# tmbdev/clstm

Hardware: AMD Instinct MI355X
Metric: text-line images/sec (fwd+bwd+CTC), 100-unit BiLSTM H=48 T~200 (higher is better)
Workload: dtype f32 (operand-exact split): forward, recurrences, CTC, decode in f32 arithmetic; the backward weight-gradient / softmax-backward products take their f32 operands split EXACTLY into three bf16 terms each (x1 + x2 + x3 = x) and sum the six bf16-MFMA products of weight >= 2^-16 in f32 -- what is dropped

## Files before the change

### clstm_amd/csrc/dbgopt.h

```cpp
#pragma once
#include <cstdlib>
#include <cstring>
#include <map>
#include <stdexcept>
#include <string>

namespace clstm {
struct DbgOptDef { const char* name; int dflt; };
inline constexpr DbgOptDef DBG_OPTS[] = {
    {"gemm_stag", 2},
    {"bwd_c32", 1},
    {"rec_x3", 1},
    {"pack_tiles", 1},
    {"fuse_wx", 1},
    {"gemm_b16mc", 1},
    {"dw_x3", 1},
    {"gemm_x3", 1},
    {"split_terms", 3},
    {"xd_prologue", 1},
    {"fwd_mfma", 1},
    {"bwd_mfma", 1},
    {"bwd_mfma_fused", 1},
    {"ctc_float", 0},
    {"peer_two_phase", 1},
};
inline const DbgOptDef* dbg_opt_def(const char* name) {
  for (const DbgOptDef& o : DBG_OPTS)
    if (strcmp(o.name, name) == 0) return &o;
  return nullptr;
}
inline std::map<std::string, int>& dbg_opts() {
  static std::map<std::string, int> m = [] {
    std::map<std::string, int> r;
    const char* e = getenv("CLSTM_DEBUG");
    if (e) {
      std::string s(e);
      size_t i = 0;
      while (i < s.size()) {
        size_t j = s.find(',', i);
        if (j == std::string::npos) j = s.size();
        const std::string kv = s.substr(i, j - i);
        const size_t eq = kv.find('=');
        if (!kv.empty()) {
          const std::string name = kv.substr(0, eq);
          if (eq == std::string::npos || !dbg_opt_def(name.c_str()))
            throw std::runtime_error("CLSTM_DEBUG: unknown option '" + name + "' (clstm_amd/csrc/dbgopt.h lists them as name=value)");
          r[name] = atoi(kv.c_str() + eq + 1);
        }
        i = j + 1;
      }
    }
    return r;
// ... 12 lines not shown
```

### clstm_amd/csrc/gemm_dw.h

```cpp
#pragma once
#include <type_traits>
#include "gemm_bf16.h"

namespace clstm {

struct DwSlab {
  int tile_begin, ntiles;
  int need_it;
  int dir;
  int out_z;
  int pad[3];
};

struct XdArgs {
  GemmOperand A;
  GemmOperand B;
  float* out; int ld;
  int K;
};

struct GemmDwArgs {
  const float* S; long long sdir; int lds; long long s_elems;
  const float* D; int M; int no4; long long d_elems;
  const int* ktab;
  int ntiles_max;
  const DwSlab* slabs;
  int nslabs;
  const int* prog;
  const int* line_off;
  int bs, prog_base, ndir;
  float* partial;
  int R, Cn;
  unsigned gx, gy;
  int* timeouts;
  int* minprog;
  int tcap;
  int* done;
  int done_target;
  long long* trace;
  int trace_base;
  const float* xS; int xlds; long long xs_elems;
  const float* xD; int xM; long long xd_elems;
  const int* xtab; const DwSlab* xslabs; int xnslabs;
  float* xpartial; int xR, xCn; unsigned xgx, xgy;
  int x3;
  int terms;
  XdArgs xd;
};

constexpr int DW_PF = 3;
constexpr int DW_STAB_MAX = 256;
// ... 337 lines not shown
```

### clstm_amd/csrc/lstm_bwd_dw.h

```cpp
#pragma once
#include "gemm_dw.h"
#include "lstm_seq.h"
#include "lstm_xd_prologue.h"

namespace clstm {

constexpr int DW_FUSED_STAB_ENTRIES = 1024;
static_assert(DW_FUSED_STAB_ENTRIES >= DW_STAB_MAX, "the items' k-tile table fits");
static_assert(xd_smem_floats(2) <= dw_img_floats(2) && xd_smem_floats(3) <= dw_img_floats(3), "the recurrence role's x.d prologue stages in the items' carve");

template <int NK4, int KU, int NT>
__global__ __launch_bounds__(64 * NK4) CLSTM_TWO_WAVES_PER_SIMD void lstm_bwd_dw_kernel(LstmSeqArgs a, GemmDwArgs g, int nrec) {
  __shared__ __attribute__((aligned(16))) float gsm[dw_img_floats(NT) + 2 * DW_FUSED_STAB_ENTRIES];
  if ((int)blockIdx.x < nrec) {
#ifndef CLSTM_HIP_EMU
    __builtin_amdgcn_s_setprio(3);
#endif
    const long long t0 = g.trace ? wall_clock() : 0;
    const int bl = (int)blockIdx.x % a.bs;
    const int b = a.order ? a.order[bl] : bl, dir = (int)blockIdx.x / a.bs;
    if constexpr (NT >= 2) {
      if (g.xd.A.p) xd_prologue<NT, xd_maxu(NK4)>(gsm, g.xd, a.line_off, b, dir, a.no);
    }
    lstm_bwd_body<NK4, KU>(a, b, dir);
    if (g.done && threadIdx.x == 0) atomic_add_i32(g.done, 1);
    if (g.trace && threadIdx.x == 0) { g.trace[blockIdx.x * 4] = t0; g.trace[blockIdx.x * 4 + 2] = wall_clock(); }
  } else {
    if (threadIdx.x >= 256) return;
    gemm_dw_body<NT>(g, gsm, blockIdx.x - (unsigned)nrec);
  }
}

}
```

### clstm_amd/csrc/lstm_seq.h

```cpp
#pragma once
#include <type_traits>
#include "devintrin.h"

namespace clstm {

struct LstmSeqArgs {
  const float* Rpk;
  float* G;
  float* C;
  float* H;
  int ldh, hofs;
  const float* dH;
  float* D;
  const int* line_off;
  const int* order;
  int no;
  int ndir;
  float* S;
  int lds, sofs;
  long long sdir;
  long long* prof;
  long long prog_off;
  int prog_base;
  int bs;
// ... 213 lines not shown
    step(t, gxA, rdyA, rdA, wrA, kaA0, kaA1, kaA2, kaB0, kaB1, kaB2);
    step(t + 1, gxB, rdyB, rdB, wrB, kaB0, kaB1, kaB2, kaA0, kaA1, kaA2);
  }
  if (t < T) {
    step(t, gxA, rdyA, rdA, wrA, kaA0, kaA1, kaA2, kaB0, kaB1, kaB2);
    if constexpr (!EARLY || STAG) flush(t, kaA0, kaA1, kaA2, report_tag);
  } else {
    if constexpr (!EARLY || STAG) flush(t - 1, kaB0, kaB1, kaB2, report_tag);
  }
  if constexpr (STAG && EARLY) __syncthreads();
  };
  if constexpr (FUSED) {
    if (wave_uniform(wave) == 3) run(std::true_type{}, std::true_type{}, std::false_type{});
    else if (early) run(std::true_type{}, std::false_type{}, std::false_type{});
    else if (wave_uniform(wave) == (nthreads >> 6) - 1) run(std::false_type{}, std::false_type{}, std::true_type{});
    else run(std::false_type{}, std::false_type{}, std::false_type{});
    drain_vmem();
    __syncthreads();
    if (tid == 0) store_i32_wt(reinterpret_cast<int*>(a.H + a.prog_off) + ((size_t)dir * a.bs + b) * PROG_STRIDE, a.prog_base + T);
  } else {
    if (early) run(std::true_type{}, std::false_type{}, std::false_type{}); else run(std::false_type{}, std::false_type{}, std::false_type{});
  }
#ifdef CLSTM_LSTM_PROF
  if (a.prof && b == 0 && dir == 0 && lane == 0)
    for (int k = 0; k < 12; k++) a.prof[wave * 12 + k] = pacc[k];
#endif
}
#undef LSTM_PIN3
template <int NK4, int KU, bool SAVE = true>
__global__ __launch_bounds__(64 * NK4) CLSTM_TWO_WAVES_PER_SIMD void lstm_fwd_kernel(LstmSeqArgs a) {
  lstm_fwd_body<NK4, KU, false, SAVE>(a, a.order ? a.order[blockIdx.x] : (int)blockIdx.x, blockIdx.y, nullptr);
}

template <int NK4, int KU>
DEVFN void lstm_bwd_body(const LstmSeqArgs& a, const int b, const int dir) {
  constexpr int SLP = 4 * NK4;
  constexpr int QS = SLP + ((NK4 & 1) ? 0 : 4);
  constexpr int DB = 16 * QS;
  float* lds = dyn_smem<float>();
  const int tid = threadIdx.x, lane = tid & 63, wave = tid >> 6;
  const int nthreads = blockDim.x;
  const int no = a.no, nd = a.ndir;
  const int SL = (4 * no + 15) / 16;
  const int js = lane & 15;
  const int g = lane & 3, cell = wave * 16 + (lane >> 2);
  const bool valid = cell < no;

  f32x2 wb01[SLP], wb23[SLP];
  {
    const float* rp = a.Rpk + (size_t)dir * 4 * SLP * nthreads + tid;
#pragma unroll
    for (int pp = 0; pp < SLP; pp++) {
      wb01[pp] = (f32x2){rp[(size_t)(0 * SLP + pp) * nthreads], rp[(size_t)(1 * SLP + pp) * nthreads]};
      wb23[pp] = (f32x2){rp[(size_t)(2 * SLP + pp) * nthreads], rp[(size_t)(3 * SLP + pp) * nthreads]};
    }
  }
  for (int i = tid; i < 2 * DB + 4; i += nthreads) lds[i] = 0.0f;

  const int off = a.line_off[b];
  const int T = a.line_off[b + 1] - off;
  if (T <= 0) {
    if (a.prog_off >= 0 && tid == 0) {
      store_i32_wt(reinterpret_cast<int*>(a.D + a.prog_off) + ((size_t)dir * a.bs + b) * PROG_STRIDE, a.prog_base);
    }
    return;
  }
  const int pidx = g * no + cell;
  const int dslot = (pidx / SL) * QS + (pidx % SL);
  const unsigned gstride4 = (unsigned)nd * 4 * no * 4, cstride4 = (unsigned)nd * no * 4;
  const BufF32 gbuf = make_buf(a.G + (size_t)off * (gstride4 / 4), (size_t)T * gstride4);
  const bool report = a.prog_off >= 0;
  const bool tagl = report && tid == nthreads - 1;
  const long long prog_rel = a.prog_off + ((long long)dir * a.bs + b) * PROG_STRIDE - (long long)off * (gstride4 / 4);
  const BufF32 dbuf = make_buf(a.D + (size_t)off * (gstride4 / 4), report ? (size_t)(prog_rel + 1) * 4 : (size_t)T * gstride4);
  const BufF32 cbuf = make_buf(a.C + (size_t)off * (cstride4 / 4), (size_t)T * cstride4);
  const BufF32 hbuf = make_buf(a.dH + (size_t)off * (cstride4 / 4), (size_t)T * cstride4);
  const unsigned gl = valid ? ((unsigned)dir * 4 * no + cell * 4 + g) * 4u : BUF_OOB_BASE;
  const unsigned ptag = (unsigned)(prog_rel * 4);
  const unsigned cl = valid ? ((unsigned)dir * no + cell) * 4u : BUF_OOB_BASE;
  auto fr = [&](int s) -> unsigned {
    const int sc = s > 0 ? s : 0;
    return (unsigned)(dir == 0 ? sc : T - 1 - sc);
  };
  const float* rdA = lds + js * QS;
  const float* rdB = lds + DB + js * QS;
  float* wrA = valid ? lds + DB + dslot : lds + 2 * DB;
  float* wrB = valid ? lds + dslot : lds + 2 * DB;
  const bool gb1 = (g & 2) != 0, gb0 = (g & 1) != 0;

  struct Ops { float act, dh, cc; };
  Ops X0, X1, X2;
  X0.act = buf_load(gbuf, gl + fr(T - 1) * gstride4); X1.act = buf_load(gbuf, gl + fr(T - 2) * gstride4);
  X0.dh = buf_load(hbuf, cl + fr(T - 1) * cstride4);  X1.dh = buf_load(hbuf, cl + fr(T - 2) * cstride4);
  X0.cc = buf_load(cbuf, cl + fr(T - 1) * cstride4);  X1.cc = buf_load(cbuf, T >= 2 ? cl + fr(T - 2) * cstride4 : BUF_OOB);
  X2.act = X2.dh = X2.cc = 0.0f;
  float dc_carry = 0.0f;
  float ka0 = 0.f, ka1 = 0.f, ka2 = 0.f;
  __syncthreads();
  auto step = [&](const int s, Ops& cur, const Ops& nxt, Ops& ld, const float* dq, float* dw, float& ka, float& kprev) {
    KEEP_ALIVE(ka);
    ld.act = buf_load(gbuf, gl + fr(s - 2) * gstride4);
    ld.dh = buf_load(hbuf, cl + fr(s - 2) * cstride4);
    ld.cc = buf_load(cbuf, s >= 2 ? cl + fr(s - 2) * cstride4 : BUF_OOB);
    const float actr = cur.act;
    const float deriv = fmaf(-actr, actr, g == 3 ? 1.0f : actr);
    const float th = tanh_fast(cur.cc);
    const float gth = mul_quad_bcast<2>(actr, fmaf(-th, th, 1.0f));
    float c_m1 = nxt.cc;
    OPAQUE(c_m1);
    const float mir = quad_mirror(actr);
    const float mid = gb0 ? c_m1 : th;
    float fb = deriv * (gb0 == gb1 ? mir : mid);
    OPAQUE(fb);
    f32x2 a01 = splat2(0.0f), a23 = splat2(0.0f);
    float4 dv[NK4];
#pragma unroll
    for (int j = 0; j < NK4; j++) dv[j] = *reinterpret_cast<const float4*>(dq + 4 * j);
    SCHED_FENCE();
    buf_store_wt(dbuf, s + 1 < T ? (tagl ? ptag : gl + fr(s + 1) * gstride4) : BUF_OOB, kprev);
    SCHED_FENCE();
#pragma unroll
    for (int j = 0; j < NK4; j++) {
      if (4 * j < KU) { a01 = fma2(wb01[4 * j], splat2(dv[j].x), a01); a23 = fma2(wb23[4 * j], splat2(dv[j].x), a23); }
      if (4 * j + 1 < KU) { a01 = fma2(wb01[4 * j + 1], splat2(dv[j].y), a01); a23 = fma2(wb23[4 * j + 1], splat2(dv[j].y), a23); }
      if (4 * j + 2 < KU) { a01 = fma2(wb01[4 * j + 2], splat2(dv[j].z), a01); a23 = fma2(wb23[4 * j + 2], splat2(dv[j].z), a23); }
      if (4 * j + 3 < KU) { a01 = fma2(wb01[4 * j + 3], splat2(dv[j].w), a01); a23 = fma2(wb23[4 * j + 3], splat2(dv[j].w), a23); }
    }
    const float k0 = a01[0] + row_ror<8>(a23[0]);
    const float k1 = a01[1] + row_ror<8>(a23[1]);
    float k = k0 + row_half_mirror(k1);
    k += quad_xor1(k);
    k += quad_xor2(k);
    const float dh = cur.dh + k;
    const float dc = dc_carry + gth * dh;
    dc_carry = mul_quad_bcast_old<1>(actr, dc);
    const float delta = (g == 2 ? dh : dc) * fb;
    const float sdat = tagl ? __builtin_bit_cast(float, a.prog_base + (T - 1 - s) - 3) : delta;
    *dw = delta;
    ka = sdat;
    __syncthreads();
  };
  int s = T - 1;
  for (; s >= 5; s -= 6) {
    step(s, X0, X1, X2, rdA, wrA, ka0, ka2);
    step(s - 1, X1, X2, X0, rdB, wrB, ka1, ka0);
    step(s - 2, X2, X0, X1, rdA, wrA, ka2, ka1);
    step(s - 3, X0, X1, X2, rdB, wrB, ka0, ka2);
    step(s - 4, X1, X2, X0, rdA, wrA, ka1, ka0);
    step(s - 5, X2, X0, X1, rdB, wrB, ka2, ka1);
  }
  if (s >= 0) step(s, X0, X1, X2, rdA, wrA, ka0, ka2);
  if (s >= 1) step(s - 1, X1, X2, X0, rdB, wrB, ka1, ka0);
  if (s >= 2) step(s - 2, X2, X0, X1, rdA, wrA, ka2, ka1);
  if (s >= 3) step(s - 3, X0, X1, X2, rdB, wrB, ka0, ka2);
  if (s >= 4) step(s - 4, X1, X2, X0, rdA, wrA, ka1, ka0);
  {
    const int r = (T - 1) % 3;
    const float last = r == 0 ? ka0 : r == 1 ? ka1 : ka2;
    buf_store_wt(dbuf, tagl ? ptag : gl + fr(0) * gstride4, last);
  }
  if (report) {
    drain_vmem();
    __syncthreads();
    if (tagl) buf_store_wt(dbuf, ptag, __builtin_bit_cast(float, a.prog_base + T));
  }
}
template <int NK4, int KU>
__global__ __launch_bounds__(64 * NK4) CLSTM_TWO_WAVES_PER_SIMD void lstm_bwd_kernel(LstmSeqArgs a) {
  lstm_bwd_body<NK4, KU>(a, a.order ? a.order[blockIdx.x] : (int)blockIdx.x, blockIdx.y);
}

}
```

### clstm_amd/csrc/lstm_xd_prologue.h

```cpp
#pragma once
#include "gemm_dw.h"
#include "lstm_seq.h"

namespace clstm {

constexpr int XD_KB = 3;
constexpr int XD_MAX_K = 32 * XD_KB;
constexpr int XD_ROWS = 32;
constexpr int XD_UNITS = XD_ROWS * XD_KB * 4;
constexpr int XD_RING = 3;
constexpr int xd_maxu(int nk4) { return nk4 <= 1 ? 6 : nk4 == 2 ? 3 : nk4 <= 7 ? 2 : 1; }
constexpr int xd_smem_floats(int nt) { return 2 * nt * XD_KB * XD_ROWS * 32 / 2; }

template <int NT, int MAXU>
DEVFN void xd_prologue(float* smem, const XdArgs& x, const int* line_off, const int b, const int dir, const int no) {
  static_assert(NT == 2 || NT == 3, "two or three bf16 terms per operand");
  unsigned short* img = reinterpret_cast<unsigned short*>(smem);
  const int tid = threadIdx.x, lane = tid & 63, wave = wave_uniform(tid >> 6);
  const int nthreads = blockDim.x;
  const int off = line_off[b];
  const int T = line_off[b + 1] - off;
  if (T <= 0) return;
  const int K = x.K;
  const BufF32 abuf = make_buf(x.A.p + (size_t)off * x.A.ld, (size_t)(x.A.elems - (long long)off * x.A.ld) * 4);
  const BufF32 bbuf = make_buf(x.B.p, (size_t)x.B.elems * 4);
  const BufF32 obuf = make_buf(x.out + (size_t)off * x.ld, (size_t)T * x.ld * 4);
  const int fk = lane >> 4, fi = lane & 15;
  constexpr int IMG = XD_ROWS * 32;
  constexpr int BUFH = NT * XD_KB * IMG;

  auto load_round = [&](const int r, f32x4 (&ra)[MAXU][2]) {
#pragma unroll
    for (int i = 0; i < MAXU; i++) {
      if (i * nthreads + (tid & ~63) >= XD_UNITS) break;
      const int u = i * nthreads + tid;
      const int row = r * XD_ROWS + u / (XD_KB * 4), ku = u % (XD_KB * 4);
      const unsigned o = u < XD_UNITS && row < T ? ((unsigned)row * (unsigned)x.A.ld + (unsigned)((ku >> 2) * 32 + (ku & 3) * 8)) * 4u : BUF_OOB_BASE;
      ra[i][0] = buf_load4(abuf, o);
      ra[i][1] = buf_load4(abuf, o + 16u);
    }
  };
  auto stage_round = [&](unsigned short* dst, const f32x4 (&ra)[MAXU][2]) {
#pragma unroll
    for (int i = 0; i < MAXU; i++) {
      if (i * nthreads + (tid & ~63) >= XD_UNITS) break;
      const int u = i * nthreads + tid;
      if (u < XD_UNITS) {
        const int row = u / (XD_KB * 4), ku = u % (XD_KB * 4), kb = ku >> 2, kk = (ku & 3) * 8;
        float v[8];
#pragma unroll
        for (int e = 0; e < 8; e++) v[e] = kb * 32 + kk + e < K ? ra[i][e >> 2][e & 3] : 0.0f;
        const int o = kb * IMG + row * 32 + (((kk >> 3) ^ gb2_sw(row)) << 3);
#pragma unroll
        for (int t = 0; t < NT; t++) {
          const u16x8 h = bf16_pack8(v);
          *reinterpret_cast<u16x8*>(dst + t * XD_KB * IMG + o) = h;
          if (t + 1 < NT) {
#pragma unroll
            for (int e = 0; e < 8; e++) v[e] -= __builtin_bit_cast(float, (unsigned)h[e] << 16);
          }
        }
      }
    }
  };

  f32x4 ring[XD_RING][MAXU][2];
#pragma unroll
  for (int p = 0; p < XD_RING; p++) {
    load_round(p, ring[p]);
    SCHED_FENCE();
  }

  const int n = wave * 16 + fi;
  const bool has_tile = wave * 16 < no;
  u16x8 bt[XD_KB][NT];
  if (has_tile) {
    const unsigned brow = n < no ? (unsigned)(dir * no + n) * (unsigned)x.B.ld * 4u : BUF_OOB_BASE;
    f32x4 rb[XD_KB][2];
#pragma unroll
    for (int kb = 0; kb < XD_KB; kb++) {
      rb[kb][0] = buf_load4(bbuf, brow + (unsigned)(kb * 32 + fk * 8) * 4u);
      rb[kb][1] = buf_load4(bbuf, brow + (unsigned)(kb * 32 + fk * 8 + 4) * 4u);
    }
#pragma unroll
    for (int kb = 0; kb < XD_KB; kb++) {
      float v[8];
#pragma unroll
      for (int i = 0; i < 8; i++) v[i] = kb * 32 + fk * 8 + i < K ? rb[kb][i >> 2][i & 3] : 0.0f;
#pragma unroll
      for (int t = 0; t < NT; t++) {
        const u16x8 h = bf16_pack8(v);
        bt[kb][t] = h;
        if (t + 1 < NT) {
#pragma unroll
          for (int i = 0; i < 8; i++) v[i] -= __builtin_bit_cast(float, (unsigned)h[i] << 16);
        }
      }
    }
  }

  const int nrounds = (T + XD_ROWS - 1) / XD_ROWS;
  const int fofs = fi * 32 + ((fk ^ gb2_sw(fi)) << 3);
  const unsigned ocol = n < no ? (unsigned)(dir * no + n) * 4u : BUF_OOB_BASE;
  auto round = [&](const int r, f32x4 (&ra)[MAXU][2]) {
    unsigned short* cur = img + (r & 1) * BUFH;
    stage_round(cur, ra);
    wait_lgkmcnt0();
    wg_barrier();
    COMPILER_MEMORY_BARRIER();
    load_round(r + XD_RING, ra);
    SCHED_FENCE();
    if (has_tile) {
      f32x4 acc[2];
#pragma unroll
      for (int m = 0; m < 2; m++)
#pragma unroll
        for (int q = 0; q < 4; q++) acc[m][q] = 0.0f;
#pragma unroll
      for (int kb = 0; kb < XD_KB; kb++) {
        u16x8 at[NT][2];
#pragma unroll
        for (int t = 0; t < NT; t++)
#pragma unroll
          for (int m = 0; m < 2; m++) at[t][m] = *reinterpret_cast<const u16x8*>(cur + (t * XD_KB + kb) * IMG + m * 16 * 32 + fofs);
#pragma unroll
        for (int w = NT - 1; w >= 0; w--)
#pragma unroll
          for (int ta = w; ta >= 0; ta--)
#pragma unroll
            for (int m = 0; m < 2; m++) acc[m] = mfma16x16x32_bf16(at[ta][m], bt[kb][w - ta], acc[m]);
      }
#pragma unroll
      for (int m = 0; m < 2; m++)
#pragma unroll
        for (int q = 0; q < 4; q++) {
          const int row = r * XD_ROWS + m * 16 + fk * 4 + q;
          buf_store(obuf, row < T ? (unsigned)row * (unsigned)x.ld * 4u + ocol : BUF_OOB_BASE, acc[m][q]);
        }
    }
  };
  for (int r = 0; r < nrounds; r += XD_RING) {
#pragma unroll
    for (int p = 0; p < XD_RING; p++)
      if (r + p < nrounds) round(r + p, ring[p]);
  }
  drain_vmem();
  __syncthreads();
}

template <int NK4, int KU, int NT>
__global__ __launch_bounds__(64 * NK4) CLSTM_TWO_WAVES_PER_SIMD void lstm_bwd_xd_kernel(LstmSeqArgs a, XdArgs x) {
  __shared__ __attribute__((aligned(16))) float xsm[xd_smem_floats(NT)];
  const int b = a.order ? a.order[blockIdx.x] : (int)blockIdx.x;
  xd_prologue<NT, xd_maxu(NK4)>(xsm, x, a.line_off, b, (int)blockIdx.y, a.no);
  lstm_bwd_body<NK4, KU>(a, b, (int)blockIdx.y);
}

}
```

### clstm_amd/csrc/net.inc

```
struct Layer {
  int ni, no, nk4, nthreads;
  bool wide = false;
  int kpf = 0, kpb = 0;
  long long nwf = 0, nwb = 0;
  PackDesc pd;
  float *Wt = nullptr, *bias = nullptr, *Rf = nullptr, *Rb = nullptr, *Rwf = nullptr, *Rwb = nullptr;
  float* Wk = nullptr;
  int wk_kp = 0, wk_njp = 0;
  DevBuf<float> dCc;
  DevBuf<unsigned short> Wmf;
  DevBuf<float> mf_scale;
  DevBuf<unsigned> mf_xmax;
  long long mf_epoch = -1;
  DevBuf<unsigned short> Wmfb;
  long long mfb_epoch = -1;
  DevBuf<int> pack_tab;
  DevBuf<int> pack_inv;
  int pack_inv_state = 0;
  unsigned short *Rbf = nullptr, *Rbb = nullptr;
  DevBuf<unsigned short> R2b, D2;
  bool r2b_ready = false;
  DevBuf<unsigned short> Hb, Db;
  DevBuf<float> Rf32;
  long long* moff = nullptr;
// ... 47 lines not shown
  bool bf16_rec = false;
  bool want_dx0 = false;
  int bs = 0, tmax = 0;
  bool src0_ready = false;
  long long N = 0;
  std::vector<int> line_off_h;
  DevBuf<int> line_off;
  std::vector<int> order_h;
  PinnedRing ring;
  const int* lo_stage = nullptr;
  bool lo_pending = false;
  void flush_line_off() {
    if (!lo_pending) return;
    hipStream_t s = stream();
    HIPCHECK(hipMemcpyAsync(line_off.p, lo_stage, (2 * bs + 1) * sizeof(int), hipMemcpyHostToDevice, s));
    ring.commit(s);
    lo_pending = false;
  }
  DevBuf<float> X, Z, Dz, dX0, partial, partial_sm, aligned, tmp;
  DevBuf<unsigned short> xbf;
  ReduceDesc sm_red{};
  DevBuf<long long> lstm_prof;
  StepGraphCache step_graphs;
  DevBuf<int> coop_sync;
  DevBuf<int> states, state_off, dec_idx, dec_cls, dec_loc, dec_cnt;
  DevBuf<float> dec_val, lat;
  DevBuf<long long> lat_off;
  Timing timing;
  static const int PROG_LINES = 2048;
  static const int PROG_WORDS = 2 * PROG_LINES * PROG_STRIDE;
  int overlap = getenv("CLSTM_OVERLAP") ? atoi(getenv("CLSTM_OVERLAP")) : 1;
  unsigned dw_done_total = 0;
  DevBuf<long long> dw_trace;
  DevBuf<int> dw_ktab, dw_slabs, dw_queue;
  std::vector<int> dw_key;
  DevBuf<int> dwx_tab;
  long long dwx_N = -1;
  int dwx_nslabs = 0, dwx_entries = 0;
  bool dwx_active = false;
  int dw_nslabs = 0, dw_slabs_per_dir = 0, dw_ntiles_max = 0;
  int prog_base = 1024;
  long long dw_launches = 0;
  Comm* comm = nullptr;
  struct HostFeed {
    hipStream_t cs = nullptr;
    hipEvent_t copied[2] = {};
    DevBuf<float> xin[2];
    void* pin[2] = {nullptr, nullptr};
    size_t pin_cap[2] = {0, 0};
    int* step_done = nullptr;
    long long steps = 0;
    bool ready = false;
  } hf;
  float* W1k = nullptr;
  int w1k_kps = 0;
  DevBuf<int> fw_items, fw_flags;
  std::vector<int> fw_key;
  int fw_npitems = 0, fw_ncitems = 0, fw_chunks = 0;
  int fw_epoch = 0, fw_prog_base = 1024;
  long long fw_launches = 0;

  hipStream_t stream() const { return g_stream; }
  bool geom_predict = false, nosave = false, in_predict = false;
  size_t fixed_bytes = 0;
  void dev_malloc(void** q, size_t bytes) { HIPCHECK(hipMalloc(q, bytes)); fixed_bytes += bytes; }

// ... 732 lines not shown
  bool dw_x3 = dbg_opt("dw_x3") != 0;
  int split_terms = dbg_opt("split_terms");
  bool gemm_x3_on = dbg_opt("gemm_x3") != 0;
  bool strict_f32 = false;
  bool rec_x3() const {
    if (bf16_gemm || bf16_rec || !gemm_x3_on) return false;
    return dbg_opt("rec_x3") != 0;
  }
  int clamp_split(long long want) const { return (int)std::max(1LL, std::min({want, (long long)(N + 63) / 64, 64LL})); }
  int pick_split_mc(int R, int Cn, int nbatch) const {
    const int th = gemm_mc_tile_rows(R);
    const long long tiles = (long long)((R + th - 1) / th) * ((Cn + 255) / 256) * nbatch;
    return clamp_split(device_cu_count() / tiles);
  }
  int pick_split(int R, int Cn, int nbatch = 1, int tile = GEMM_BT) const {
    const long long tiles = (long long)((R + tile - 1) / tile) * ((Cn + tile - 1) / tile) * nbatch;
    const long long target = tile == GEMM_BT ? 640 : 480;
    long long want = (target + tiles - 1) / tiles;
    if (tile == 256) want = device_cu_count() / tiles;
    return clamp_split(want);
  }

  bool overlap_eligible(const Layer& y) const {
    if (!overlap || y.wide || y.no % 16 == 0) return false;
    if (bs > PROG_LINES) return false;
    if ((overlap == 1) && (tmax < 64 || N < 2048)) return false;
    if ((double)y.D.cap * 4.0 >= 2147483000.0) return false;
    return overlap == 2 || y.nthreads >= 256;
  }
  BwdFamily backward_family(const Layer& y) const {
    if (!bf16_gemm && overlap_eligible(y)) return BwdFamily::Overlapped;
    return y.wide ? BwdFamily::Wide : BwdFamily::Narrow;
  }
  bool xd_in_launch() const {
    const Layer& top = L.back();
    return dwx_active && !mfma_bwd_eligible(top) && desc.nclasses <= XD_MAX_K && top.nthreads >= 64 * ((top.no + 15) / 16) &&
           top.nthreads * xd_maxu(top.nk4) >= XD_UNITS &&
           dbg_opt("xd_prologue") != 0;
  }
  XdArgs xd_args() const {
    const Layer& top = L.back();
    const int nc = desc.nclasses;
    return XdArgs{gemm_kc(Dz.p, nc, N), gemm_kc(v + sm_off + nc, nc, sm_ni, 0), top.dH.p, sm_ni, nc};
  }
  static int dw_bf16_rows(const Layer& y, int R, int Cn) { return wide_kp16_bwd(y.no) == 4 * y.no && gemm_bf16_big(R - 1, Cn) ? R - 1 : R; }
  static constexpr int DW_CHUNK = 16, DW_TAIL_PARTS = 4, DW_TAIL_CHUNKS = 2;
  void build_dw_tables() {
    if (dw_key == line_off_h && dw_nslabs > 0) return;
    std::vector<int> cb;
    for (int done = DW_CHUNK; done < tmax; done += DW_CHUNK) cb.push_back(done);
    cb.push_back(tmax);
    const int tiles_per_slab = std::min(DW_STAB_MAX, std::max(8, (int)((N / 16 + 15) / 16)));
    std::vector<std::vector<int>> tab(ndir);
    struct Sl { int tb, nt, need, dir, chunk, part; };
    std::vector<std::vector<Sl>> sl(ndir);
    for (int dir = 0; dir < ndir; dir++) {
      int cs = 0;
      for (size_t c = 0; c < cb.size(); c++) {
        const int ce = cb[c];
        const int t0 = (int)tab[dir].size() / 2;
        for (int b = 0; b < bs; b++) {
          const int off = line_off_h[b], T = line_off_h[b + 1] - off;
          if (T <= cs) continue;
          const int e = std::min(ce, T);
          const int f_lo = dir == 0 ? T - e : cs, f_hi = dir == 0 ? T - cs : e;
          for (int f = f_lo; f < f_hi; f += 16) { tab[dir].push_back(off + f); tab[dir].push_back(std::min(16, f_hi - f)); }
        }
        const int nt = (int)tab[dir].size() / 2 - t0;
        int parts = std::max(1, (nt + tiles_per_slab - 1) / tiles_per_slab);
        if (c + DW_TAIL_CHUNKS >= cb.size()) parts = std::max(parts, std::min(DW_TAIL_PARTS, std::max(1, nt / 2)));
        for (int p = 0; p < parts; p++) {
          const int a0 = t0 + (int)((long long)nt * p / parts), a1 = t0 + (int)((long long)nt * (p + 1) / parts);
          REQUIRE(a1 - a0 <= DW_STAB_MAX, "internal: weight-gradient slab longer than its LDS table");
          sl[dir].push_back(Sl{a0, a1 - a0, ce, dir, (int)c, p});
        }
        cs = ce;
// ... 3 lines not shown
    for (int dir = 1; dir < ndir; dir++) REQUIRE((int)sl[dir].size() == dw_slabs_per_dir, "internal: asymmetric slab lists");
    dw_ntiles_max = 0;
    for (int dir = 0; dir < ndir; dir++) dw_ntiles_max = std::max(dw_ntiles_max, (int)tab[dir].size() / 2);
    std::vector<DwSlab> slabs;
    for (int i = 0; i < dw_slabs_per_dir; i++)
      for (int dir = 0; dir < ndir; dir++) {
        const Sl& x = sl[dir][i];
        slabs.push_back(DwSlab{x.tb, x.nt, x.need, dir, dir * dw_slabs_per_dir + i, {0, 0, 0}});
      }
    dw_nslabs = (int)slabs.size();
    const size_t nk = (size_t)ndir * dw_ntiles_max * 2, nsw = slabs.size() * sizeof(DwSlab) / sizeof(int);
    dw_ktab.reserve(nk + 8);
    dw_slabs.reserve(nsw + 8);
    hipStream_t s = stream();
    int* stage = (int*)ring.acquire((nk + nsw) * sizeof(int));
    for (int dir = 0; dir < ndir; dir++) {
      std::fill(stage + (size_t)dir * dw_ntiles_max * 2, stage + (size_t)(dir + 1) * dw_ntiles_max * 2, 0);
      std::copy(tab[dir].begin(), tab[dir].end(), stage + (size_t)dir * dw_ntiles_max * 2);
    }
    memcpy(stage + nk, slabs.data(), nsw * sizeof(int));
    HIPCHECK(hipMemcpyAsync(dw_ktab.p, stage, nk * sizeof(int), hipMemcpyHostToDevice, s));
    HIPCHECK(hipMemcpyAsync(dw_slabs.p, stage + nk, nsw * sizeof(int), hipMemcpyHostToDevice, s));
    ring.commit(s);
    dw_key = line_off_h;
  }
  void backward_layer_overlapped(Layer& y, LstmSeqArgs a, int R, int Cn) {
    hipStream_t s = stream();
    build_dw_tables();
    const int M = ndir * 4 * y.no;
    const long long prog_off = (long long)y.D.cap - 64 - PROG_WORDS;
    REQUIRE(prog_off >= (long long)N * M, "internal: progress words overlap the deltas");
    prog_base += tmax + 64;
    dw_launches++;
    if (prog_base > (1 << 30)) prog_base = 1024;
    a.prog_off = prog_off;
    a.prog_base = prog_base;
    DevBuf<float>& partial = layer_partial(y);
    partial.reserve((size_t)ndir * dw_slabs_per_dir * R * Cn);
    GemmDwArgs g{};
    g.S = y.S.p; g.sdir = (long long)N * y.lds; g.lds = y.lds; g.s_elems = (long long)N * ndir * y.lds + 3;
    g.D = y.D.p; g.M = M; g.no4 = 4 * y.no; g.d_elems = (long long)N * M + 3;
    g.ktab = dw_ktab.p; g.ntiles_max = dw_ntiles_max; g.slabs = (const DwSlab*)dw_slabs.p; g.nslabs = dw_nslabs;
    g.prog = (const int*)(y.D.p + prog_off); g.line_off = line_off.p; g.bs = bs; g.prog_base = prog_base;
    g.partial = partial.p; g.R = R; g.Cn = Cn;
    g.gx = (unsigned)((Cn + GEMM_BT - 1) / GEMM_BT); g.gy = (unsigned)((R + GEMM_BT - 1) / GEMM_BT);
    g.timeouts = dev_err_words() + 1;
    if (!dw_queue.p) dw_queue.reserve(5 * PROG_STRIDE);
    g.ndir = ndir;
    g.minprog = dw_queue.p + PROG_STRIDE;
    g.tcap = tmax + 32;
    g.done = nullptr; g.done_target = 0;
    g.x3 = dw_x3;
    g.terms = split_terms;
    unsigned nextra = 0;
    const bool xd = &y == &L.back() && xd_in_launch();
    if (xd) { g.xd = xd_args(); g_path_count[PC_XD_PROLOGUE]++; }
    if (dwx_active && &y == &L.back()) {
      const int xR = 1 + sm_ni, xCn = desc.nclasses;
      g.xS = y.srow(); g.xlds = y.ldh; g.xs_elems = (long long)N * y.ldh + 3;
      g.xD = Dz.p; g.xM = xCn; g.xd_elems = (long long)N * xCn + 3;
      g.xtab = dwx_tab.p; g.xslabs = (const DwSlab*)(dwx_tab.p + 2 * dwx_entries); g.xnslabs = dwx_nslabs;
      g.xpartial = partial_sm.p; g.xR = xR; g.xCn = xCn;
      g.xgx = (unsigned)((xCn + GEMM_BT - 1) / GEMM_BT); g.xgy = (unsigned)((xR + GEMM_BT - 1) / GEMM_BT);
      nextra = (unsigned)dwx_nslabs * g.xgx * g.xgy;
    }
    static const char* trace_path = getenv("CLSTM_DW_TRACE");
    const size_t trace_rows = (size_t)bs * ndir + (size_t)((dw_nslabs + 7) / 8) * 8 * g.gx * g.gy + 8;
    if (trace_path) { dw_trace.reserve(trace_rows * 4); g.trace = dw_trace.p; g.trace_base = bs * ndir; }
    const unsigned nblk = 1u + nextra + (unsigned)((dw_nslabs + 7) / 8) * 8u * g.gx * g.gy;
#ifndef CLSTM_HIP_EMU
    if (mfma_bwd_fused_ok(y, g)) {
      timing.begin("lstm_bwd", s);
      g.done = nullptr; g.done_target = 0;
      const bool ok = y.no == 64 ? launch_mfma_bwd_dw_no<64>(y, a, g, nblk, s) : launch_mfma_bwd_dw_no<100>(y, a, g, nblk, s);
      timing.end(s);
      check_launch();
      if (ok) return;
    }
    if (y.nthreads >= 256 && !mfma_bwd_eligible(y)) {
      timing.begin("lstm_bwd", s);
      g.done = g.minprog + 2 * PROG_STRIDE;
      dw_done_total += (unsigned)(bs * ndir);
      g.done_target = (int)dw_done_total;
      REQUIRE(launch_lstm_bwd_dw(y.nk4, y.pd.ku, a, g, bs * ndir, nblk, y.nthreads, s), "internal: no fused instantiation");
      timing.end(s);
      if (trace_path)
        dump_trace(trace_path, dw_trace.p, trace_rows, s,
                   "# rows 0..%d: recurrence workgroups (start, -, end); then one row per (slab, tile) item: start ready done need_it; 100 MHz ticks\n", bs * ndir - 1);
      return;
    }
#endif
    timing.begin("lstm_bwd", s);
    launch_bwd_narrow(y, a, s, xd ? &g.xd : nullptr);
    timing.end(s);
    timing.begin("gemm_gates_dw", s);
    if (g.x3 && g.terms >= 3) CLSTM_LAUNCH(gemm_dw_kernel<3>, dim3(nblk), dim3(256), 0, s, g);
    else if (g.x3) CLSTM_LAUNCH(gemm_dw_kernel<2>, dim3(nblk), dim3(256), 0, s, g);
    else CLSTM_LAUNCH(gemm_dw_kernel<0>, dim3(nblk), dim3(256), 0, s, g);
    timing.end(s);
    check_launch();
  }

  void build_dwx_table() {
    if (dwx_N == N) return;
    hipStream_t s = stream();
    dwx_entries = (int)((N + 15) / 16);
    const int eps = std::min(DW_STAB_MAX, std::max(32, (dwx_entries + 63) / 64));
    dwx_nslabs = (dwx_entries + eps - 1) / eps;
    const size_t nsw = (size_t)dwx_nslabs * sizeof(DwSlab) / sizeof(int);
    dwx_tab.reserve((size_t)2 * dwx_entries + nsw + 8);
    int* stage = (int*)ring.acquire(((size_t)2 * dwx_entries + nsw) * sizeof(int));
    for (int e = 0; e < dwx_entries; e++) { stage[2 * e] = 16 * e; stage[2 * e + 1] = (int)std::min<long long>(16, N - 16LL * e); }
    DwSlab* sl = (DwSlab*)(stage + 2 * dwx_entries);
    for (int i = 0; i < dwx_nslabs; i++) sl[i] = DwSlab{eps * i, std::min(eps, dwx_entries - eps * i), 0, 0, i, {0, 0, 0}};
    for (int i = 0; i < dwx_nslabs; i++) REQUIRE(sl[i].ntiles <= DW_STAB_MAX, "internal: weight-gradient slab longer than its LDS table");
    HIPCHECK(hipMemcpyAsync(dwx_tab.p, stage, ((size_t)2 * dwx_entries + nsw) * sizeof(int), hipMemcpyHostToDevice, s));
    ring.commit(s);
    dwx_N = N;
  }
  struct ReduceTarget { bool fuse, peer; float* gdst; };
  void backward() {
    REQUIRE(N > 0, "set_batch first");
    const bool fuse = fuse_update, peer = peer_step && comm;
    fuse_update = false;
// ... 316 lines not shown
```

### clstm_amd/csrc/runtime.inc

```

static thread_local std::string g_err;
static thread_local hipStream_t g_stream = nullptr;

struct Error : std::runtime_error {
  using std::runtime_error::runtime_error;
};
#define HIPCHECK(expr)                                                                       \
  do {                                                                                       \
    hipError_t e_ = (expr);                                                                  \
    if (e_ != hipSuccess)                                                                    \
      throw Error(std::string(#expr) + " failed: " + hipGetErrorString(e_) + " (" + __FILE__ + \
                  ":" + std::to_string(__LINE__) + ")");                                     \
  } while (0)
#define REQUIRE(cond, msg)                    \
  do {                                        \
    if (!(cond)) throw Error(std::string(msg)); \
  } while (0)
#define ABI_BEGIN try {
#define ABI_END                         \
  return 0;                             \
  }                                     \
  catch (const std::exception& e) {     \
    g_err = e.what();                   \
    return 1;                           \
// ... 65 lines not shown
    return h[cur];
  }
  void commit(hipStream_t s) {
    if (cur % GROUP != GROUP - 1) return;
    const int g = cur / GROUP;
    if (!ev[g]) HIPCHECK(hipEventCreateWithFlags(&ev[g], hipEventDisableTiming));
    HIPCHECK(hipEventRecord(ev[g], s));
    busy[g] = true;
  }
  ~PinnedRing() {
    for (int i = 0; i < SLOTS / GROUP; i++)
      if (ev[i]) (void)hipEventDestroy(ev[i]);
    for (int i = 0; i < SLOTS; i++)
      if (h[i]) (void)hipHostFree(h[i]);
  }
};

struct StoreBias {
  float* out; long long ld; const float* bias;
  DEVMFN void operator()(int r, int c, float v, int) const { out[(long long)r * ld + c] = v + bias[c]; }
  DEVMFN bool vec4() const { return (ld & 3) == 0 && (((size_t)out | (size_t)bias) & 15) == 0; }
  DEVMFN void row4(int r, int c, f32x4 v, int) const {
    const f32x4 b = *reinterpret_cast<const f32x4*>(bias + c);
    f32x4 o;
    o[0] = v[0] + b[0]; o[1] = v[1] + b[1]; o[2] = v[2] + b[2]; o[3] = v[3] + b[3];
    *reinterpret_cast<f32x4*>(out + (long long)r * ld + c) = o;
  }
};
enum PathCounter {
  PC_FWD_PERSISTENT = 0, PC_BWD_PERSISTENT = 1, PC_WX_FROM_BF16 = 2, PC_DX_FROM_BF16 = 3, PC_DW_FROM_BF16 = 4, PC_FWD_FUSED = 5,
  PC_FWD_FUSED_WX = 6, PC_PEER_EXCHANGE = 7, PC_DW_X_EXTERNAL = 8, PC_BWD_C32 = 9, PC_PACKS_FOLLOW_UPDATE = 10, PC_BWD_X3 = 11,
  PC_REPLICA_CHECK = 12, PC_DW_BIAS_OUT = 13, PC_DW_DX_ONE_LAUNCH = 14, PC_MFMA_NOSAVE = 15, PC_MFMA_FWD = 16, PC_MFMA_BWD = 17,
  PC_MFMA_BWD_DW = 18, PC_INGEST_TAIL = 19, PC_INGEST_TAIL_USED = 20, PC_MFMA_ROUTED = 21 ,
  PC_LINE_NOSAVE = 22, PC_FUSED_NOSAVE = 23, PC_PEER_TWO_PHASE = 24, PC_NORMALIZED = 25, PC_XD_PROLOGUE = 26, PC_COUNT
};
static long long g_path_count[PC_COUNT];
struct StorePlain {
  float* out; long long ld;
  DEVMFN void operator()(int r, int c, float v, int) const { out[(long long)r * ld + c] = v; }
  DEVMFN bool vec4() const { return (ld & 3) == 0 && ((size_t)out & 15) == 0; }
  DEVMFN void row4(int r, int c, f32x4 v, int) const { *reinterpret_cast<f32x4*>(out + (long long)r * ld + c) = v; }
};
struct StorePartial {
  float* out; int R, Cn;
  DEVMFN void operator()(int r, int c, float v, int z) const { out[((long long)z * R + r) * Cn + c] = v; }
  DEVMFN bool vec4() const { return (Cn & 3) == 0 && ((size_t)out & 15) == 0; }
  DEVMFN void row4(int r, int c, f32x4 v, int z) const {
    *reinterpret_cast<f32x4*>(out + ((long long)z * R + r) * Cn + c) = v;
  }
};
struct StorePartialShift {
  float* out; int R, Cn;
  DEVMFN void operator()(int r, int c, float v, int z) const { out[((long long)z * R + r + 1) * Cn + c] = v; }
  DEVMFN bool vec4() const { return (Cn & 3) == 0 && ((size_t)out & 15) == 0; }
  DEVMFN void row4(int r, int c, f32x4 v, int z) const { *reinterpret_cast<f32x4*>(out + ((long long)z * R + r + 1) * Cn + c) = v; }
};
struct StorePartialRot {
  float* out; int R, Cn;
  DEVMFN void operator()(int r, int c, float v, int z) const { out[((long long)z * R + (r + 1 == R ? 0 : r + 1)) * Cn + c] = v; }
  DEVMFN bool vec4() const { return (Cn & 3) == 0 && ((size_t)out & 15) == 0; }
  DEVMFN void row4(int r, int c, f32x4 v, int z) const {
    *reinterpret_cast<f32x4*>(out + ((long long)z * R + (r + 1 == R ? 0 : r + 1)) * Cn + c) = v;
  }
};
#ifndef GEMM_BK_DW
#define GEMM_BK_DW 16
#endif
// ... 433 lines not shown
```

Before: 229,900.

## Overlap x.d prologue with backward recurrence via producer workgroups and ready flags

Previously each recurrence workgroup computed the whole x.d product (softmax delta times output weights) before starting its backward recurrence. In the new mode each recurrence workgroup computes only the first round of rows it needs. Extra producer workgroups in the same launch compute the remaining rounds and publish progress through per-line ready words. Wave 0 of the recurrence polls those words before it consumes later rows, which takes the prologue off the serial critical path. In exchange it adds polling, write-through stores, extra workgroups that compete for CUs, and a timeout fallback. The mode is gated on the CU count and is the new default.

```diff
diff --git a/clstm_amd/csrc/dbgopt.h b/clstm_amd/csrc/dbgopt.h
--- a/clstm_amd/csrc/dbgopt.h
+++ b/clstm_amd/csrc/dbgopt.h
@@ -17,7 +17,7 @@
     {"dw_x3", 1},
     {"gemm_x3", 1},
     {"split_terms", 3},
-    {"xd_prologue", 1},
+    {"xd_prologue", 2},
     {"fwd_mfma", 1},
     {"bwd_mfma", 1},
     {"bwd_mfma_fused", 1},
diff --git a/clstm_amd/csrc/gemm_dw.h b/clstm_amd/csrc/gemm_dw.h
--- a/clstm_amd/csrc/gemm_dw.h
+++ b/clstm_amd/csrc/gemm_dw.h
@@ -17,6 +17,7 @@
   GemmOperand B;
   float* out; int ld;
   int K;
+  int* ready; int ready0;
 };
 
 struct GemmDwArgs {
diff --git a/clstm_amd/csrc/lstm_bwd_dw.h b/clstm_amd/csrc/lstm_bwd_dw.h
--- a/clstm_amd/csrc/lstm_bwd_dw.h
+++ b/clstm_amd/csrc/lstm_bwd_dw.h
@@ -19,15 +19,31 @@
     const long long t0 = g.trace ? wall_clock() : 0;
     const int bl = (int)blockIdx.x % a.bs;
     const int b = a.order ? a.order[bl] : bl, dir = (int)blockIdx.x / a.bs;
+    bool producers = false;
     if constexpr (NT >= 2) {
-      if (g.xd.A.p) xd_prologue<NT, xd_maxu(NK4)>(gsm, g.xd, a.line_off, b, dir, a.no);
+      if (g.xd.A.p) {
+        producers = g.xd.ready != nullptr;
+        if (producers) xd_own_round<NT, xd_maxu(NK4)>(gsm, g.xd, a.line_off, b, dir, a.no);
+        else xd_prologue<NT, xd_maxu(NK4)>(gsm, g.xd, a.line_off, b, dir, a.no);
+      }
     }
-    lstm_bwd_body<NK4, KU>(a, b, dir);
+    const long long t1 = g.trace ? wall_clock() : 0;
+    if constexpr (NT >= 2) {
+      if (producers) lstm_bwd_body<NK4, KU, true>(a, b, dir, g.xd.ready + ((size_t)dir * a.bs + b) * PROG_STRIDE, g.xd.ready0);
+      else lstm_bwd_body<NK4, KU>(a, b, dir);
+    } else lstm_bwd_body<NK4, KU>(a, b, dir);
     if (g.done && threadIdx.x == 0) atomic_add_i32(g.done, 1);
-    if (g.trace && threadIdx.x == 0) { g.trace[blockIdx.x * 4] = t0; g.trace[blockIdx.x * 4 + 2] = wall_clock(); }
+    if (g.trace && threadIdx.x == 0) { g.trace[blockIdx.x * 4] = t0; g.trace[blockIdx.x * 4 + 1] = t1; g.trace[blockIdx.x * 4 + 2] = wall_clock(); }
   } else {
+    unsigned blk = blockIdx.x - (unsigned)nrec;
+    if constexpr (NT >= 2) {
+      if (g.xd.ready) {
+        if (blk >= 1u && blk <= (unsigned)nrec) { xd_item<NT, xd_maxu(NK4)>(gsm, g.xd, a.line_off, a.order, a.bs, (int)blk - 1, a.no); return; }
+        if (blk > (unsigned)nrec) blk -= (unsigned)nrec;
+      }
+    }
     if (threadIdx.x >= 256) return;
-    gemm_dw_body<NT>(g, gsm, blockIdx.x - (unsigned)nrec);
+    gemm_dw_body<NT>(g, gsm, blk);
   }
 }
 
diff --git a/clstm_amd/csrc/lstm_seq.h b/clstm_amd/csrc/lstm_seq.h
--- a/clstm_amd/csrc/lstm_seq.h
+++ b/clstm_amd/csrc/lstm_seq.h
@@ -269,8 +269,8 @@
   lstm_fwd_body<NK4, KU, false, SAVE>(a, a.order ? a.order[blockIdx.x] : (int)blockIdx.x, blockIdx.y, nullptr);
 }
 
-template <int NK4, int KU>
-DEVFN void lstm_bwd_body(const LstmSeqArgs& a, const int b, const int dir) {
+template <int NK4, int KU, bool XDP = false>
+DEVFN void lstm_bwd_body(const LstmSeqArgs& a, const int b, const int dir, const int* xdw = nullptr, const int xd0 = 0) {
   constexpr int SLP = 4 * NK4;
   constexpr int QS = SLP + ((NK4 & 1) ? 0 : 4);
   constexpr int DB = 16 * QS;
@@ -325,20 +325,26 @@
   float* wrB = valid ? lds + dslot : lds + 2 * DB;
   const bool gb1 = (g & 2) != 0, gb0 = (g & 1) != 0;
 
-  struct Ops { float act, dh, cc; };
+  struct Ops { float act, dh, cc; int rdy; };
+  auto hload = [&](unsigned o) -> float { return XDP ? buf_load_wt(hbuf, o) : buf_load(hbuf, o); };
   Ops X0, X1, X2;
   X0.act = buf_load(gbuf, gl + fr(T - 1) * gstride4); X1.act = buf_load(gbuf, gl + fr(T - 2) * gstride4);
-  X0.dh = buf_load(hbuf, cl + fr(T - 1) * cstride4);  X1.dh = buf_load(hbuf, cl + fr(T - 2) * cstride4);
+  X0.dh = hload(cl + fr(T - 1) * cstride4);           X1.dh = hload(cl + fr(T - 2) * cstride4);
   X0.cc = buf_load(cbuf, cl + fr(T - 1) * cstride4);  X1.cc = buf_load(cbuf, T >= 2 ? cl + fr(T - 2) * cstride4 : BUF_OOB);
   X2.act = X2.dh = X2.cc = 0.0f;
+  X0.rdy = X1.rdy = X2.rdy = xd0;
   float dc_carry = 0.0f;
   float ka0 = 0.f, ka1 = 0.f, ka2 = 0.f;
+  bool xd_gave_up = false;
   __syncthreads();
+  auto run = [&](auto chk_t) {
+  constexpr bool CHK = decltype(chk_t)::value;
   auto step = [&](const int s, Ops& cur, const Ops& nxt, Ops& ld, const float* dq, float* dw, float& ka, float& kprev) {
     KEEP_ALIVE(ka);
     ld.act = buf_load(gbuf, gl + fr(s - 2) * gstride4);
-    ld.dh = buf_load(hbuf, cl + fr(s - 2) * cstride4);
+    ld.dh = hload(cl + fr(s - 2) * cstride4);
     ld.cc = buf_load(cbuf, s >= 2 ? cl + fr(s - 2) * cstride4 : BUF_OOB);
+    if constexpr (CHK) ld.rdy = load_i32_wt(xdw);
     const float actr = cur.act;
     const float deriv = fmaf(-actr, actr, g == 3 ? 1.0f : actr);
     const float th = tanh_fast(cur.cc);
@@ -375,6 +381,17 @@
     const float sdat = tagl ? __builtin_bit_cast(float, a.prog_base + (T - 1 - s) - 3) : delta;
     *dw = delta;
     ka = sdat;
+    if constexpr (CHK) {
+      const int itn = T + 2 - s < T ? T + 2 - s : T - 1;
+      const int need = itn >> 5;
+      if (need > 0 && !xd_gave_up && __builtin_expect(wave_uniform(cur.rdy) - xd0 < need, 0)) {
+        int polls = 0;
+        while (wave_uniform(load_i32_wt(xdw)) - xd0 < need) {
+          poll_pause();
+          if (++polls > (1 << 20)) { if (lane == 0) atomic_add_i32(a.timeouts, 1); xd_gave_up = true; break; }
+        }
+      }
+    }
     __syncthreads();
   };
   int s = T - 1;
@@ -391,6 +408,10 @@
   if (s >= 2) step(s - 2, X2, X0, X1, rdA, wrA, ka2, ka1);
   if (s >= 3) step(s - 3, X0, X1, X2, rdB, wrB, ka0, ka2);
   if (s >= 4) step(s - 4, X1, X2, X0, rdA, wrA, ka1, ka0);
+  };
+  if constexpr (XDP) {
+    if (wave_uniform(wave) == 0) run(std::true_type{}); else run(std::false_type{});
+  } else run(std::false_type{});
   {
     const int r = (T - 1) % 3;
     const float last = r == 0 ? ka0 : r == 1 ? ka1 : ka2;
diff --git a/clstm_amd/csrc/lstm_xd_prologue.h b/clstm_amd/csrc/lstm_xd_prologue.h
--- a/clstm_amd/csrc/lstm_xd_prologue.h
+++ b/clstm_amd/csrc/lstm_xd_prologue.h
@@ -12,8 +12,9 @@
 constexpr int xd_maxu(int nk4) { return nk4 <= 1 ? 6 : nk4 == 2 ? 3 : nk4 <= 7 ? 2 : 1; }
 constexpr int xd_smem_floats(int nt) { return 2 * nt * XD_KB * XD_ROWS * 32 / 2; }
 
-template <int NT, int MAXU>
-DEVFN void xd_prologue(float* smem, const XdArgs& x, const int* line_off, const int b, const int dir, const int no) {
+template <int NT, int MAXU, bool WT = false>
+DEVFN void xd_rounds(float* smem, const XdArgs& x, const int* line_off, const int b, const int dir, const int no,
+                     const int row0, const int rstep, const int nr, int* word = nullptr, const int word0 = 0) {
   static_assert(NT == 2 || NT == 3, "two or three bf16 terms per operand");
   unsigned short* img = reinterpret_cast<unsigned short*>(smem);
   const int tid = threadIdx.x, lane = tid & 63, wave = wave_uniform(tid >> 6);
@@ -34,8 +35,8 @@
     for (int i = 0; i < MAXU; i++) {
       if (i * nthreads + (tid & ~63) >= XD_UNITS) break;
       const int u = i * nthreads + tid;
-      const int row = r * XD_ROWS + u / (XD_KB * 4), ku = u % (XD_KB * 4);
-      const unsigned o = u < XD_UNITS && row < T ? ((unsigned)row * (unsigned)x.A.ld + (unsigned)((ku >> 2) * 32 + (ku & 3) * 8)) * 4u : BUF_OOB_BASE;
+      const int row = row0 + r * rstep + u / (XD_KB * 4), ku = u % (XD_KB * 4);
+      const unsigned o = u < XD_UNITS && r < nr && (unsigned)row < (unsigned)T ? ((unsigned)row * (unsigned)x.A.ld + (unsigned)((ku >> 2) * 32 + (ku & 3) * 8)) * 4u : BUF_OOB_BASE;
       ra[i][0] = buf_load4(abuf, o);
       ra[i][1] = buf_load4(abuf, o + 16u);
     }
@@ -99,15 +100,20 @@
     }
   }
 
-  const int nrounds = (T + XD_ROWS - 1) / XD_ROWS;
   const int fofs = fi * 32 + ((fk ^ gb2_sw(fi)) << 3);
   const unsigned ocol = n < no ? (unsigned)(dir * no + n) * 4u : BUF_OOB_BASE;
   auto round = [&](const int r, f32x4 (&ra)[MAXU][2]) {
     unsigned short* cur = img + (r & 1) * BUFH;
     stage_round(cur, ra);
     wait_lgkmcnt0();
+    if constexpr (WT) {
+      if (word) drain_vmem();
+    }
     wg_barrier();
     COMPILER_MEMORY_BARRIER();
+    if constexpr (WT) {
+      if (word && r > 0 && tid == 0) store_i32_wt(word, word0 + r);
+    }
     load_round(r + XD_RING, ra);
     SCHED_FENCE();
     if (has_tile) {
@@ -134,18 +140,46 @@
       for (int m = 0; m < 2; m++)
 #pragma unroll
         for (int q = 0; q < 4; q++) {
-          const int row = r * XD_ROWS + m * 16 + fk * 4 + q;
-          buf_store(obuf, row < T ? (unsigned)row * (unsigned)x.ld * 4u + ocol : BUF_OOB_BASE, acc[m][q]);
+          const int row = row0 + r * rstep + m * 16 + fk * 4 + q;
+          const unsigned o = (unsigned)row < (unsigned)T ? (unsigned)row * (unsigned)x.ld * 4u + ocol : BUF_OOB_BASE;
+          if constexpr (WT) buf_store_wt(obuf, o, acc[m][q]);
+          else buf_store(obuf, o, acc[m][q]);
         }
     }
   };
-  for (int r = 0; r < nrounds; r += XD_RING) {
+  for (int r = 0; r < nr; r += XD_RING) {
 #pragma unroll
     for (int p = 0; p < XD_RING; p++)
-      if (r + p < nrounds) round(r + p, ring[p]);
+      if (r + p < nr) round(r + p, ring[p]);
   }
   drain_vmem();
   __syncthreads();
+  if constexpr (WT) {
+    if (word && tid == 0) store_i32_wt(word, word0 + nr);
+  }
+}
+
+template <int NT, int MAXU>
+DEVFN void xd_prologue(float* smem, const XdArgs& x, const int* line_off, const int b, const int dir, const int no) {
+  const int T = line_off[b + 1] - line_off[b];
+  xd_rounds<NT, MAXU>(smem, x, line_off, b, dir, no, 0, XD_ROWS, (T + XD_ROWS - 1) / XD_ROWS);
+}
+
+DEVFN int xd_visit_rounds(const int T) { return (T + XD_ROWS - 1) / XD_ROWS; }
+template <int NT, int MAXU>
+DEVFN void xd_own_round(float* smem, const XdArgs& x, const int* line_off, const int b, const int dir, const int no) {
+  const int T = line_off[b + 1] - line_off[b];
+  xd_rounds<NT, MAXU, true>(smem, x, line_off, b, dir, no, dir == 0 ? T - XD_ROWS : 0, 0, 1);
+}
+template <int NT, int MAXU>
+DEVFN void xd_item(float* smem, const XdArgs& x, const int* line_off, const int* order, const int bs, const int i, const int no) {
+  const int bl = i % bs, dir = i / bs;
+  const int b = order ? order[bl] : bl;
+  const int T = line_off[b + 1] - line_off[b];
+  const int nv = xd_visit_rounds(T);
+  if (nv <= 1) return;
+  xd_rounds<NT, MAXU, true>(smem, x, line_off, b, dir, no, dir == 0 ? T - 2 * XD_ROWS : XD_ROWS, dir == 0 ? -XD_ROWS : XD_ROWS, nv - 1,
+                            x.ready + ((size_t)dir * bs + b) * PROG_STRIDE, x.ready0);
 }
 
 template <int NK4, int KU, int NT>
diff --git a/clstm_amd/csrc/net.inc b/clstm_amd/csrc/net.inc
--- a/clstm_amd/csrc/net.inc
+++ b/clstm_amd/csrc/net.inc
@@ -103,6 +103,7 @@
   int overlap = getenv("CLSTM_OVERLAP") ? atoi(getenv("CLSTM_OVERLAP")) : 1;
   unsigned dw_done_total = 0;
   DevBuf<long long> dw_trace;
+  DevBuf<int> xd_ready;
   DevBuf<int> dw_ktab, dw_slabs, dw_queue;
   std::vector<int> dw_key;
   DevBuf<int> dwx_tab;
@@ -901,16 +902,23 @@
     if (!bf16_gemm && overlap_eligible(y)) return BwdFamily::Overlapped;
     return y.wide ? BwdFamily::Wide : BwdFamily::Narrow;
   }
-  bool xd_in_launch() const {
+  int xd_mode() const {
     const Layer& top = L.back();
-    return dwx_active && !mfma_bwd_eligible(top) && desc.nclasses <= XD_MAX_K && top.nthreads >= 64 * ((top.no + 15) / 16) &&
-           top.nthreads * xd_maxu(top.nk4) >= XD_UNITS &&
-           dbg_opt("xd_prologue") != 0;
-  }
+    const int opt = dbg_opt("xd_prologue");
+    const bool ok = dwx_active && !mfma_bwd_eligible(top) && desc.nclasses <= XD_MAX_K && top.nthreads >= 64 * ((top.no + 15) / 16) &&
+                    top.nthreads * xd_maxu(top.nk4) >= XD_UNITS &&
+                    opt != 0;
+    if (!ok) return 0;
+#ifndef CLSTM_HIP_EMU
+    if (opt >= 2 && top.nthreads >= 256 && (long long)bs * ndir * 2 <= device_cu_count()) return 2;
+#endif
+    return 1;
+  }
+  bool xd_in_launch() const { return xd_mode() != 0; }
   XdArgs xd_args() const {
     const Layer& top = L.back();
     const int nc = desc.nclasses;
-    return XdArgs{gemm_kc(Dz.p, nc, N), gemm_kc(v + sm_off + nc, nc, sm_ni, 0), top.dH.p, sm_ni, nc};
+    return XdArgs{gemm_kc(Dz.p, nc, N), gemm_kc(v + sm_off + nc, nc, sm_ni, 0), top.dH.p, sm_ni, nc, nullptr, 0};
   }
   static int dw_bf16_rows(const Layer& y, int R, int Cn) { return wide_kp16_bwd(y.no) == 4 * y.no && gemm_bf16_big(R - 1, Cn) ? R - 1 : R; }
   static constexpr int DW_CHUNK = 16, DW_TAIL_PARTS = 4, DW_TAIL_CHUNKS = 2;
@@ -980,7 +988,8 @@
     REQUIRE(prog_off >= (long long)N * M, "internal: progress words overlap the deltas");
     prog_base += tmax + 64;
     dw_launches++;
-    if (prog_base > (1 << 30)) prog_base = 1024;
+    const bool prog_base_wrapped = prog_base > (1 << 30);
+    if (prog_base_wrapped) prog_base = 1024;
     a.prog_off = prog_off;
     a.prog_base = prog_base;
     DevBuf<float>& partial = layer_partial(y);
@@ -1002,7 +1011,17 @@
     g.terms = split_terms;
     unsigned nextra = 0;
     const bool xd = &y == &L.back() && xd_in_launch();
-    if (xd) { g.xd = xd_args(); g_path_count[PC_XD_PROLOGUE]++; }
+    const int xdm = &y == &L.back() ? xd_mode() : 0;
+    if (xd) { g.xd = xd_args(); g_path_count[xdm == 2 ? PC_XD_PRODUCERS : PC_XD_PROLOGUE]++; }
+    if (xdm == 2) {
+      const size_t nw = (size_t)ndir * bs * PROG_STRIDE;
+      if (nw > xd_ready.cap || prog_base_wrapped) {
+        xd_ready.reserve(nw);
+        HIPCHECK(hipMemsetAsync(xd_ready.p, 0, xd_ready.cap * sizeof(int), s));
+      }
+      g.xd.ready = xd_ready.p; g.xd.ready0 = prog_base;
+      a.timeouts = g.timeouts;
+    }
     if (dwx_active && &y == &L.back()) {
       const int xR = 1 + sm_ni, xCn = desc.nclasses;
       g.xS = y.srow(); g.xlds = y.ldh; g.xs_elems = (long long)N * y.ldh + 3;
@@ -1015,7 +1034,7 @@
     static const char* trace_path = getenv("CLSTM_DW_TRACE");
     const size_t trace_rows = (size_t)bs * ndir + (size_t)((dw_nslabs + 7) / 8) * 8 * g.gx * g.gy + 8;
     if (trace_path) { dw_trace.reserve(trace_rows * 4); g.trace = dw_trace.p; g.trace_base = bs * ndir; }
-    const unsigned nblk = 1u + nextra + (unsigned)((dw_nslabs + 7) / 8) * 8u * g.gx * g.gy;
+    const unsigned nblk = 1u + (xdm == 2 ? (unsigned)(bs * ndir) : 0u) + nextra + (unsigned)((dw_nslabs + 7) / 8) * 8u * g.gx * g.gy;
 #ifndef CLSTM_HIP_EMU
     if (mfma_bwd_fused_ok(y, g)) {
       timing.begin("lstm_bwd", s);
@@ -1034,10 +1053,11 @@
       timing.end(s);
       if (trace_path)
         dump_trace(trace_path, dw_trace.p, trace_rows, s,
-                   "# rows 0..%d: recurrence workgroups (start, -, end); then one row per (slab, tile) item: start ready done need_it; 100 MHz ticks\n", bs * ndir - 1);
+                   "# rows 0..%d: recurrence workgroups (start, x.d prologue returned, end); then one row per (slab, tile) item: start ready done need_it; 100 MHz ticks\n", bs * ndir - 1);
       return;
     }
 #endif
+    REQUIRE(xdm != 2, "internal: the producer form of x.d outside the one-launch form");
     timing.begin("lstm_bwd", s);
     launch_bwd_narrow(y, a, s, xd ? &g.xd : nullptr);
     timing.end(s);
diff --git a/clstm_amd/csrc/runtime.inc b/clstm_amd/csrc/runtime.inc
--- a/clstm_amd/csrc/runtime.inc
+++ b/clstm_amd/csrc/runtime.inc
@@ -121,7 +121,7 @@
   PC_FWD_FUSED_WX = 6, PC_PEER_EXCHANGE = 7, PC_DW_X_EXTERNAL = 8, PC_BWD_C32 = 9, PC_PACKS_FOLLOW_UPDATE = 10, PC_BWD_X3 = 11,
   PC_REPLICA_CHECK = 12, PC_DW_BIAS_OUT = 13, PC_DW_DX_ONE_LAUNCH = 14, PC_MFMA_NOSAVE = 15, PC_MFMA_FWD = 16, PC_MFMA_BWD = 17,
   PC_MFMA_BWD_DW = 18, PC_INGEST_TAIL = 19, PC_INGEST_TAIL_USED = 20, PC_MFMA_ROUTED = 21 ,
-  PC_LINE_NOSAVE = 22, PC_FUSED_NOSAVE = 23, PC_PEER_TWO_PHASE = 24, PC_NORMALIZED = 25, PC_XD_PROLOGUE = 26, PC_COUNT
+  PC_LINE_NOSAVE = 22, PC_FUSED_NOSAVE = 23, PC_PEER_TWO_PHASE = 24, PC_NORMALIZED = 25, PC_XD_PROLOGUE = 26, PC_XD_PRODUCERS = 27, PC_COUNT
 };
 static long long g_path_count[PC_COUNT];
 struct StorePlain {
```

Result: faster. 232,900 (median of 6 runs) (+1.3%).
